# FearL0rd/ComfyUI-ParallelAnything

Hardware: AMD Instinct MI355X
Metric: images_per_s (whole-job; sec/it in ms_per_step), flux 1024^2 batch=8 (higher is better)
Workload: dtype bf16; 1 GPU; model=FLUX.1-dev-class MMDiT 12B, global_batch=8, resolution=1024, seq_len=4608, parallelism=dp1

## Files before the change

comfyui_parallelanything_amd/models/layers.py:

```python
from __future__ import annotations

import math
from dataclasses import dataclass
from typing import Tuple

import torch
from torch import nn

from .. import ops


class FusedGELU(nn.Module):

    def forward(self, x):
        return ops.gelu_tanh(x)


class GELULinear(nn.Module):

    def __init__(self, in_features: int, out_features: int):
        super().__init__()
        self.lin = nn.Linear(in_features, out_features, bias=True)

    def forward(self, x):
# ... 287 lines not shown
            qkv = qkv_lin.mm_fp8(x8, s_used)
            y_up = mlp_lin.mm_fp8(x8, s_used)
            if (hasattr(self.linear2_mlp, "gelu_quant")
                    and ops.hip_available("gelu_fp8")):
                mlp_fp8 = self.linear2_mlp.gelu_quant(y_up)
                mlp_act = None
            else:
                mlp_act = ops.gelu_tanh(y_up)
        else:
            x_in = ops.layer_norm_mod(x, mod.scale, mod.shift)
            qkv = self.linear1_qkv(x_in)
            mlp_act = self.linear1_mlp(x_in)
        qkv = qkv.unflatten(-1, (3, self.num_heads, -1))
        q, k, v = qkv.unbind(2)
        ops.qk_norm_rope_(
            q, k, self.norm.query_norm.scale, self.norm.key_norm.scale, pe
        )
        attn = ops.attention_bshd(q, k, v, self.attn.scale,
                                  key_mask=key_mask).flatten(2)
        if mlp_fp8 is not None:
            out = self.linear2_attn(attn) + self.linear2_mlp.mm_fp8(*mlp_fp8)
        elif x.is_cuda and isinstance(self.linear2_mlp, nn.Linear):
            acc = self.linear2_attn(attn).reshape(-1, hidden)
            out = torch.addmm(
                acc, mlp_act.reshape(-1, self.mlp_dim),
                self.linear2_mlp.weight.t(),
            ).reshape(B, S, hidden)
        else:
            out = self.linear2_attn(attn) + self.linear2_mlp(mlp_act)
        return ops.gate_residual(x, mod.gate, out)


class LastLayer(nn.Module):

    def __init__(self, hidden: int, out_dim: int):
        super().__init__()
        self.ada_lin = nn.Linear(hidden, 2 * hidden, bias=True)
        self.linear = nn.Linear(hidden, out_dim, bias=True)

    def forward(self, x, vec):
        shift, scale = self.ada_lin(torch.nn.functional.silu(vec)).chunk(2, dim=-1)
        return self.linear(ops.layer_norm_mod(x, scale, shift))


def _mod_outs(chunked):
    return ModOut(*chunked[:3]), (ModOut(*chunked[3:]) if len(chunked) == 6 else None)


# ... 31 lines not shown
```

comfyui_parallelanything_amd/ops/__init__.py:

```python
from __future__ import annotations

import glob
import importlib.util
import logging
import math
import os
from dataclasses import dataclass
from typing import Optional

import torch

from . import reference

log = logging.getLogger("parallelanything.ops")

_EXT = None
_EXT_TRIED = False
_ALLOW_EAGER = os.environ.get("PA_ALLOW_EAGER", "0") == "1"
_WARNED: set = set()
_NATIVE16 = (torch.bfloat16, torch.float16)


def _load_ext():
    global _EXT, _EXT_TRIED
# ... 107 lines not shown
    _refuse_unless(img.device == txt.device,
                   f"{op}: img is on {img.device}, txt on {txt.device}")
    for name, w in zip(("wq_t", "wk_t", "wq_i", "wk_i"), weights):
        _check_norm_weight(op, name, w, D, txt)
    _check_cs(op, cs, T + img.shape[1], D, txt)



def rms_norm(x: torch.Tensor, weight=None, eps: float = 1e-6) -> torch.Tensor:
    if x.is_cuda:
        ext = _require_ext("rms_norm")
        if ext is not None:
            return ext.rms_norm(x.contiguous(),
                                weight.contiguous() if weight is not None else None,
                                eps)
    return reference.rms_norm(x, weight, eps)


def layer_norm_mod(x, scale, shift, eps: float = 1e-6) -> torch.Tensor:
    if x.is_cuda:
        ext = _require_ext("layer_norm_mod")
        if ext is not None:
            if scale.dim() == x.dim() - 1:
                return ext.layer_norm_mod(
                    x.contiguous(), scale.contiguous(), shift.contiguous(), eps
                )
            _unsupported("layer_norm_mod", "per-token modulation")
    return reference.layer_norm_mod(x, scale, shift, eps)


def gate_residual(residual, gate, x) -> torch.Tensor:
    if x.dim() == 3 and gate.dim() == 2 and not x.is_cuda:
        _refuse_unless(
            tuple(gate.shape) == (x.shape[0], x.shape[2]),
            f"gate_residual: gate must be [B, D] = [{x.shape[0]}, "
            f"{x.shape[2]}], got {list(gate.shape)}")
        _refuse_unless(
            residual.shape == x.shape,
            f"gate_residual: residual {list(residual.shape)} must have x's "
            f"shape {list(x.shape)}")
        _refuse_unless(residual.dtype == x.dtype and gate.dtype == x.dtype,
                       "gate_residual: residual and gate dtypes must match "
                       "x's")
    if x.is_cuda:
        ext = _require_ext("gate_residual")
        if ext is not None and gate.dim() == x.dim() - 1:
            return ext.gate_residual(residual.contiguous(), gate.contiguous(),
                                     x.contiguous())
    return reference.gate_residual(residual, gate, x)


def group_norm_silu(x, num_groups: int, weight=None, bias=None,
                    eps: float = 1e-6) -> torch.Tensor:
    if x.is_cuda:
        ext = _require_ext("group_norm_silu")
        if ext is not None:
            if x.dim() == 4 and (x.shape[1] % num_groups) == 0:
                return ext.group_norm_silu(
                    x.contiguous(), int(num_groups),
                    weight.contiguous() if weight is not None else None,
                    bias.contiguous() if bias is not None else None,
                    eps,
                )
            _unsupported("group_norm_silu", f"dim={x.dim()}")
    return reference.group_norm_silu(x, num_groups, weight, bias, eps)


_GN_NHWC_MAX_C = 4096
_GN_NHWC_MAX_GROUPS = 256

# ... 448 lines not shown
```

comfyui_parallelanything_amd/ops/hip/common.h:

```cpp
#pragma once

#include <torch/extension.h>
#include <vector>
#include <ATen/ATen.h>
#include <c10/hip/HIPStream.h>

#include <hip/hip_runtime.h>
#include <hip/hip_bf16.h>
#include <hip/hip_fp16.h>
#include <hip/hip_fp8.h>

#define PA_DEV __device__ __forceinline__

using bf16 = __hip_bfloat16;
typedef __attribute__((ext_vector_type(8))) short short8;
typedef __attribute__((ext_vector_type(4))) short short4v;
typedef __attribute__((ext_vector_type(2))) float f32x2;

static constexpr int WAVE = 64;

PA_DEV float bf2f(bf16 v) { return __bfloat162float(v); }
PA_DEV bf16 f2bf(float v) { return __float2bfloat16(v); }

typedef __attribute__((ext_vector_type(16))) float f32x16;
// ... 76 lines not shown

static bool is_elem16(at::ScalarType t) {
    return t == at::kBFloat16 || t == at::kHalf;
}

#define PA_WITH_ELEM16(ST, ...)                                               \
    do {                                                                      \
        if ((ST) == at::kBFloat16) { using E = bf16; __VA_ARGS__; }           \
        else { using E = _Float16; __VA_ARGS__; }                             \
    } while (0)

#define PA_WITH_DTYPE(OP, ST, ...)                                            \
    do {                                                                      \
        if ((ST) == at::kBFloat16) { using T = bf16; __VA_ARGS__; }           \
        else if ((ST) == at::kHalf) { using T = _Float16; __VA_ARGS__; }      \
        else if ((ST) == at::kFloat) { using T = float; __VA_ARGS__; }        \
        else TORCH_CHECK(false, OP ": unsupported dtype ", (ST),              \
                         " (bf16, fp16 or fp32)");                            \
    } while (0)

static int grid_1d(long n) {
    return (int)std::min<long>((n + 255) / 256, 4096);
}
```

comfyui_parallelanything_amd/ops/hip/elementwise.h:

```cpp
#pragma once

template <typename T>
__global__ void gate_residual_kernel(const T* __restrict__ res,
                                     const T* __restrict__ gate,
                                     const T* __restrict__ x,
                                     T* __restrict__ out,
                                     long total, int S, int D) {
    const long stride = (long)gridDim.x * blockDim.x;
    for (long i = (long)blockIdx.x * blockDim.x + threadIdx.x; i < total; i += stride) {
        const long d = i % D;
        const long b = i / ((long)S * D);
        out[i] = (T)((float)res[i] + (float)gate[b * D + d] * (float)x[i]);
    }
}

template <typename E>
__global__ void gate_residual_vec_kernel(const E* __restrict__ res,
                                         const E* __restrict__ gate,
                                         const E* __restrict__ x,
                                         E* __restrict__ out,
                                         long total8, int S, int DV) {
    using EL = Elem16<E>;
    const long stride = (long)gridDim.x * blockDim.x;
    const short8* rv = reinterpret_cast<const short8*>(res);
    const short8* gv = reinterpret_cast<const short8*>(gate);
    const short8* xv = reinterpret_cast<const short8*>(x);
    short8* ov = reinterpret_cast<short8*>(out);
    for (long i = (long)blockIdx.x * blockDim.x + threadIdx.x; i < total8;
         i += stride) {
        const long dv = i % DV;
        const long b = i / ((long)S * DV);
        short8 r = rv[i], g = gv[b * DV + dv], xx = xv[i], o;
#pragma unroll
        for (int j = 0; j < 8; ++j) {
            float f = EL::ld((unsigned short)r[j]) +
                      EL::ld((unsigned short)g[j]) *
                          EL::ld((unsigned short)xx[j]);
            o[j] = (short)EL::st(f);
        }
        ov[i] = o;
    }
}

at::Tensor gate_residual(at::Tensor res, at::Tensor gate, at::Tensor x) {
    CHECK_GPU(x);
    TORCH_CHECK(x.dim() == 3 && gate.dim() == 2,
                "gate_residual: x [B,S,D], gate [B,D]");
    TORCH_CHECK(gate.size(0) == x.size(0) && gate.size(1) == x.size(2),
                "gate_residual: gate must be [B, D] = [", x.size(0), ", ",
                x.size(2), "], got ", gate.sizes());
    TORCH_CHECK(res.sizes() == x.sizes(), "gate_residual: residual ",
                res.sizes(), " must have x's shape ", x.sizes());
    CHECK_SAME_DEVICE(res, x);
    CHECK_SAME_DEVICE(gate, x);
    CHECK_SAME_DTYPE(res, x);
    CHECK_SAME_DTYPE(gate, x);
    if (x.numel() == 0) return at::empty(x.sizes(), x.options());
    auto rc = res.contiguous();
    auto gc = gate.contiguous();
    auto xc = x.contiguous();
    auto out = at::empty_like(xc);
    const long total = xc.numel();
    const int S = (int)xc.size(1), D = (int)xc.size(2);
    const int blocks = grid_1d(total);
    const auto st = xc.scalar_type();
    if (is_elem16(st) && (D % 8) == 0) {
        PA_WITH_ELEM16(st, hipLaunchKernelGGL(
            gate_residual_vec_kernel<E>, dim3(blocks), dim3(256), 0,
            cur_stream(), (const E*)rc.data_ptr(), (const E*)gc.data_ptr(),
            (const E*)xc.data_ptr(), (E*)out.data_ptr(), total / 8, S, D / 8));
    } else {
        PA_WITH_DTYPE("gate_residual", st, hipLaunchKernelGGL(
            gate_residual_kernel<T>, dim3(blocks), dim3(256), 0,
            cur_stream(), (const T*)rc.data_ptr(), (const T*)gc.data_ptr(),
            (const T*)xc.data_ptr(), (T*)out.data_ptr(), total, S, D));
    }
    return out;
}

template <bool kTail = false>
PA_DEV float gelu_tanh_f32(float f) {
    const float c = 0.7978845608028654f * (f + 0.044715f * f * f * f);
    const float En = __builtin_amdgcn_exp2f(-2.8853900817779268f * fabsf(c));
    const float r = __builtin_amdgcn_rcpf(1.f + En);
    return f * (c >= 0.f ? r : (kTail ? En * r : 1.f - r));
}

template <typename E>
__global__ void gelu_tanh_vec_kernel(const E* __restrict__ x,
                                     E* __restrict__ out, long total8,
                                     long rows, long w8, long in_stride8) {
    using EL = Elem16<E>;
    const long stride = (long)gridDim.x * blockDim.x;
    const short8* xv = reinterpret_cast<const short8*>(x);
    short8* ov = reinterpret_cast<short8*>(out);
    for (long i = (long)blockIdx.x * blockDim.x + threadIdx.x; i < total8;
         i += stride) {
        const long src = (in_stride8 == w8)
// ... 198 lines not shown
```

comfyui_parallelanything_amd/ops/hip/norm.h:

```cpp
#pragma once

template <typename T>
__global__ void rms_norm_kernel(const T* __restrict__ x, const T* __restrict__ w,
                                T* __restrict__ out, int D, float eps) {
    const long row = blockIdx.x;
    const T* xr = x + row * (long)D;
    T* yr = out + row * (long)D;
    __shared__ float scratch[8];

    float acc = 0.f;
    for (int i = threadIdx.x; i < D; i += blockDim.x) {
        float v = (float)xr[i];
        acc += v * v;
    }
    float ssq = block_reduce_sum<256>(acc, scratch);
    const float rrms = rsqrtf(ssq / (float)D + eps);
    for (int i = threadIdx.x; i < D; i += blockDim.x) {
        float v = (float)xr[i] * rrms;
        if (w != nullptr) v *= (float)w[i];
        yr[i] = (T)v;
    }
}

template <typename E>
// ... 98 lines not shown
        PA_WITH_ELEM16(st, hipLaunchKernelGGL(
            rms_norm_row_kernel<E>, dim3((unsigned)((rows + 3) / 4)),
            dim3(256), 0, cur_stream(), (const E*)xc.data_ptr(),
            (const E*)wptr, (E*)out.data_ptr(), rows, D, (float)eps));
    } else if (is_elem16(st) && (D % 8) == 0) {
        PA_WITH_ELEM16(st, hipLaunchKernelGGL(
            rms_norm_vec_kernel<E>, dim3((unsigned)rows), dim3(256), 0,
            cur_stream(), (const E*)xc.data_ptr(), (const E*)wptr,
            (E*)out.data_ptr(), D, (float)eps));
    } else {
        PA_WITH_DTYPE("rms_norm", st, hipLaunchKernelGGL(
            rms_norm_kernel<T>, dim3((unsigned)rows), dim3(256), 0,
            cur_stream(), (const T*)xc.data_ptr(), (const T*)wptr,
            (T*)out.data_ptr(), D, (float)eps));
    }
    return out;
}

template <typename T>
__global__ void layer_norm_mod_kernel(const T* __restrict__ x,
                                      const T* __restrict__ scale,
                                      const T* __restrict__ shift,
                                      T* __restrict__ out,
                                      int S, int D, float eps) {
    const long row = blockIdx.x;
    const long b = row / S;
    const T* xr = x + row * (long)D;
    const T* sc = scale + b * (long)D;
    const T* sh = shift + b * (long)D;
    T* yr = out + row * (long)D;
    __shared__ float scratch[8];

    float s1 = 0.f, s2 = 0.f;
    for (int i = threadIdx.x; i < D; i += blockDim.x) {
        float v = (float)xr[i];
        s1 += v;
        s2 += v * v;
    }
    float mean = block_reduce_sum<256>(s1, scratch) / (float)D;
    float var = block_reduce_sum<256>(s2, scratch) / (float)D - mean * mean;
    float corr = 0.f;
    if constexpr (sizeof(T) == 4) {
        float sd = 0.f, sq = 0.f;
        for (int i = threadIdx.x; i < D; i += blockDim.x) {
            float d = (float)xr[i] - mean;
            sd += d;
            sq += d * d;
        }
        corr = block_reduce_sum<256>(sd, scratch) / (float)D;
        var = block_reduce_sum<256>(sq, scratch) / (float)D - corr * corr;
    }
    const float rstd = rsqrtf(fmaxf(var, 0.f) + eps);
// ... 47 lines not shown
    }
    __syncthreads();
    s1 = (scratch[0] + scratch[2]) + (scratch[4] + scratch[6]);
    s2 = (scratch[1] + scratch[3]) + (scratch[5] + scratch[7]);
    const double inv_d = 1.0 / (double)D;
    const double m = s1 * inv_d;
    mean = (float)m;
    rstd = rsqrtf(fmaxf((float)(s2 * inv_d - m * m), 0.f) + eps);
}

template <typename EL>
PA_DEV float ln_modulate(short x, short scale, short shift, float mean,
                         float rstd) {
    float f = (EL::ld((unsigned short)x) - mean) * rstd;
    return f * (1.f + EL::ld((unsigned short)scale)) +
           EL::ld((unsigned short)shift);
}

template <typename E>
__global__ void layer_norm_mod_vec_kernel(const E* __restrict__ x,
                                          const E* __restrict__ scale,
                                          const E* __restrict__ shift,
                                          E* __restrict__ out,
                                          int S, int D, float eps) {
    using EL = Elem16<E>;
    const long row = blockIdx.x;
    const long b = row / S;
    const short8* xr = reinterpret_cast<const short8*>(x + row * (long)D);
    const short8* sc = reinterpret_cast<const short8*>(scale + b * (long)D);
    const short8* sh = reinterpret_cast<const short8*>(shift + b * (long)D);
    short8* yr = reinterpret_cast<short8*>(out + row * (long)D);
    const int DV = D / 8;
    __shared__ float scratch[8];

    float mean, rstd;
    ln_row_stats<EL>(xr, D, eps, scratch, mean, rstd);
    for (int i = threadIdx.x; i < DV; i += blockDim.x) {
        short8 v = xr[i], a = sc[i], c = sh[i], o;
#pragma unroll
        for (int j = 0; j < 8; ++j)
            o[j] = (short)EL::st(ln_modulate<EL>(v[j], a[j], c[j], mean, rstd));
        yr[i] = o;
    }
}

at::Tensor layer_norm_mod(at::Tensor x, at::Tensor scale, at::Tensor shift,
                          double eps) {
    CHECK_GPU(x);
    TORCH_CHECK(x.dim() == 3, "layer_norm_mod expects [B, S, D]");
    auto xc = x.contiguous();
    auto sc = scale.contiguous();
    auto sh = shift.contiguous();
    TORCH_CHECK(sc.sizes() == sh.sizes() && sc.dim() == 2, "scale/shift [B, D]");
    auto out = at::empty_like(xc);
    const int B = (int)xc.size(0), S = (int)xc.size(1), D = (int)xc.size(2);
    dim3 grid((unsigned)((long)B * S));
    const auto st = xc.scalar_type();
    CHECK_SAME_DTYPE(scale, x);
    CHECK_SAME_DTYPE(shift, x);
    if (is_elem16(st) && (D % 8) == 0) {
        PA_WITH_ELEM16(st, hipLaunchKernelGGL(
            layer_norm_mod_vec_kernel<E>, grid, dim3(256), 0, cur_stream(),
            (const E*)xc.data_ptr(), (const E*)sc.data_ptr(),
            (const E*)sh.data_ptr(), (E*)out.data_ptr(), S, D, (float)eps));
    } else {
        PA_WITH_DTYPE("layer_norm_mod", st, hipLaunchKernelGGL(
            layer_norm_mod_kernel<T>, grid, dim3(256), 0, cur_stream(),
            (const T*)xc.data_ptr(), (const T*)sc.data_ptr(),
            (const T*)sh.data_ptr(), (T*)out.data_ptr(), S, D, (float)eps));
    }
    return out;
}

template <typename T>
__global__ void group_norm_silu_kernel(const T* __restrict__ x,
                                       const float* __restrict__ w,
                                       const float* __restrict__ bias,
                                       T* __restrict__ out,
                                       int C, long HW, int G, float eps) {
    const int b = blockIdx.x / G;
    const int g = blockIdx.x % G;
    const int cpg = C / G;
    const long base = ((long)b * C + (long)g * cpg) * HW;
    const long n = (long)cpg * HW;
    __shared__ float scratch[8];

    float s1 = 0.f, s2 = 0.f;
    for (long i = threadIdx.x; i < n; i += blockDim.x) {
        float v = (float)x[base + i];
        s1 += v;
        s2 += v * v;
    }
// ... 51 lines not shown
```

comfyui_parallelanything_amd/ops/hip/qk_pack.h:

```cpp
#pragma once

template <typename EL>
PA_DEV unsigned int rms_rope_pair(unsigned int u, float w0, float w1, float c,
                                  float s, bool act, int D, float eps) {
    float a0 = EL::ld((unsigned short)(u & 0xffff));
    float a1 = EL::ld((unsigned short)(u >> 16));
    const float ss = wave_reduce_sum(act ? a0 * a0 + a1 * a1 : 0.f);
    const float rr = rsqrtf(ss / (float)D + eps);
    a0 = a0 * rr * w0;
    a1 = a1 * rr * w1;
    return (unsigned int)EL::st(a0 * c - a1 * s) |
           ((unsigned int)EL::st(a0 * s + a1 * c) << 16);
}

static void check_cs_table(const char* op, const at::Tensor& cs, long S, long D,
                           const at::Tensor& ref) {
    TORCH_CHECK(cs.dim() == 3 && cs.size(0) == S && cs.size(1) == D / 2 &&
                cs.size(2) == 2, op, ": cs must be [S, D/2, 2] = [", S, ", ",
                D / 2, ", 2], got ", cs.sizes());
    TORCH_CHECK(cs.device() == ref.device(), op, ": cs is on ", cs.device(),
                ", the activations on ", ref.device());
}

static void check_norm_weight(const char* op, const char* name,
                              const at::Tensor& w, long D,
                              const at::Tensor& ref) {
    TORCH_CHECK(w.dim() == 1 && w.size(0) == D, op, ": ", name,
                " must be [D] = [", D, "], got ", w.sizes());
    TORCH_CHECK(w.scalar_type() == ref.scalar_type(), op, ": ", name,
                " dtype (", w.scalar_type(), ") must match the activations (",
                ref.scalar_type(), ")");
    TORCH_CHECK(w.device() == ref.device(), op, ": ", name, " is on ",
                w.device(), ", the activations on ", ref.device());
}

template <typename E>
__global__ void qk_norm_rope_kernel(E* __restrict__ q, E* __restrict__ k,
                                    const E* __restrict__ wq,
                                    const E* __restrict__ wk,
                                    const float* __restrict__ cs,
                                    int S, int H, int D,
                                    long q_bs, long q_hs, long q_ss,
                                    long k_bs, long k_hs, long k_ss,
                                    long n_rows, float eps) {
    using EL = Elem16<E>;
    constexpr int RPW = 4;
    const int lane = threadIdx.x & 63;
    const long wave = ((long)blockIdx.x * blockDim.x + threadIdx.x) >> 6;
    const int pairs = D / 2;
    const bool act = lane < pairs;
    const int ln = act ? lane : 0;

    unsigned int uq[RPW], uk[RPW];
    unsigned int* qp[RPW];
    unsigned int* kp[RPW];
    float cvec[RPW], svec[RPW];
    const unsigned int uwq = reinterpret_cast<const unsigned int*>(wq)[ln];
    const unsigned int uwk = reinterpret_cast<const unsigned int*>(wk)[ln];
#pragma unroll
    for (int i = 0; i < RPW; ++i) {
        const long row = wave * RPW + i;
        const long rr = row < n_rows ? row : n_rows - 1;
        const long b = rr / ((long)S * H);
        const long sh = rr % ((long)S * H);
        const int sj = (int)(sh / H);
        const int h = (int)(sh % H);
        qp[i] = reinterpret_cast<unsigned int*>(
            q + b * q_bs + (long)sj * q_ss + (long)h * q_hs);
        kp[i] = reinterpret_cast<unsigned int*>(
            k + b * k_bs + (long)sj * k_ss + (long)h * k_hs);
        uq[i] = qp[i][ln];
        uk[i] = kp[i][ln];
        cvec[i] = cs[((long)sj * pairs + ln) * 2 + 0];
        svec[i] = cs[((long)sj * pairs + ln) * 2 + 1];
    }
    const float wq0 = EL::ld((unsigned short)(uwq & 0xffff));
    const float wq1 = EL::ld((unsigned short)(uwq >> 16));
    const float wk0 = EL::ld((unsigned short)(uwk & 0xffff));
    const float wk1 = EL::ld((unsigned short)(uwk >> 16));
#pragma unroll
    for (int i = 0; i < RPW; ++i) {
        if (wave * RPW + i >= n_rows) break;
        const unsigned int oq = rms_rope_pair<EL>(
            uq[i], wq0, wq1, cvec[i], svec[i], act, D, eps);
        if (act) qp[i][lane] = oq;
        const unsigned int ok = rms_rope_pair<EL>(
            uk[i], wk0, wk1, cvec[i], svec[i], act, D, eps);
        if (act) kp[i][lane] = ok;
    }
}

void qk_norm_rope_(at::Tensor q, at::Tensor k, at::Tensor wq, at::Tensor wk,
                   at::Tensor cs, double eps) {
    CHECK_GPU(q);
    TORCH_CHECK(q.dim() == 4 && k.dim() == 4, "qk_norm_rope_: [B,S,H,D] views");
    TORCH_CHECK(is_elem16(q.scalar_type()),
                "qk_norm_rope_: bf16 or fp16 only, got ", q.scalar_type());
    CHECK_SAME_DTYPE(k, q);
    CHECK_SAME_DEVICE(k, q);
    const int B = (int)q.size(0), S = (int)q.size(1), H = (int)q.size(2),
              D = (int)q.size(3);
    TORCH_CHECK(D % 2 == 0 && D <= 128, "qk_norm_rope_: D must be even, <=128");
    TORCH_CHECK(k.sizes() == q.sizes(), "qk_norm_rope_: k ", k.sizes(),
                " must have q's shape ", q.sizes());
    check_norm_weight("qk_norm_rope_", "wq", wq, D, q);
    check_norm_weight("qk_norm_rope_", "wk", wk, D, q);
    check_cs_table("qk_norm_rope_", cs, S, D, q);
    const long rows = (long)B * S * H;
    if (rows == 0 || D == 0) return;
    TORCH_CHECK(q.stride(3) == 1 && k.stride(3) == 1,
                "qk_norm_rope_: last dim contiguous");
    auto csf = cs.to(at::kFloat).contiguous();
    auto wqc = wq.contiguous();
    auto wkc = wk.contiguous();
    const long blocks = (((rows + 3) / 4) * 64 + 255) / 256;
    PA_WITH_ELEM16(q.scalar_type(), hipLaunchKernelGGL(
        qk_norm_rope_kernel<E>, dim3((unsigned)blocks), dim3(256), 0,
        cur_stream(), (E*)q.data_ptr(), (E*)k.data_ptr(),
        (const E*)wqc.data_ptr(), (const E*)wkc.data_ptr(),
        csf.data_ptr<float>(), S, H, D,
        q.stride(0), q.stride(2), q.stride(1),
        k.stride(0), k.stride(2), k.stride(1), rows, (float)eps));
}

template <typename E>
__global__ void pack_joint_qkv_kernel(
    const E* __restrict__ txt, const E* __restrict__ img,
    const E* __restrict__ wq_t, const E* __restrict__ wk_t,
    const E* __restrict__ wq_i, const E* __restrict__ wk_i,
    const float* __restrict__ cs,
    E* __restrict__ oq, E* __restrict__ ok, E* __restrict__ ov,
    int T, int Si, int H, int D,
    long t_bs, long t_ss, long t_qs, long t_hs,
    long i_bs, long i_ss, long i_qs, long i_hs,
    long n_rows, float eps) {
    using EL = Elem16<E>;
    constexpr int RPW = 4;
    const int lane = threadIdx.x & 63;
    const long wave = ((long)blockIdx.x * blockDim.x + threadIdx.x) >> 6;
    const int S = T + Si;
    const int pairs = D / 2;
    const bool act = lane < pairs;
    const int ln = act ? lane : 0;

    unsigned int uq[RPW], uk[RPW], uv[RPW], uwq[RPW], uwk[RPW];
    long obase[RPW];
    float cvec[RPW], svec[RPW];
#pragma unroll
    for (int i = 0; i < RPW; ++i) {
        const long row = wave * RPW + i;
        const long rr = row < n_rows ? row : n_rows - 1;
        const long b = rr / ((long)S * H);
        const long sh = rr % ((long)S * H);
        const int sj = (int)(sh / H);
        const int h = (int)(sh % H);
        const bool is_txt = sj < T;
        const E* src = is_txt
            ? txt + b * t_bs + (long)sj * t_ss + (long)h * t_hs
            : img + b * i_bs + (long)(sj - T) * i_ss + (long)h * i_hs;
        const long qs = is_txt ? t_qs : i_qs;
        uq[i] = reinterpret_cast<const unsigned int*>(src)[ln];
        uk[i] = reinterpret_cast<const unsigned int*>(src + qs)[ln];
        uv[i] = reinterpret_cast<const unsigned int*>(src + 2 * qs)[ln];
        uwq[i] = reinterpret_cast<const unsigned int*>(is_txt ? wq_t : wq_i)[ln];
        uwk[i] = reinterpret_cast<const unsigned int*>(is_txt ? wk_t : wk_i)[ln];
        cvec[i] = cs[((long)sj * pairs + ln) * 2 + 0];
        svec[i] = cs[((long)sj * pairs + ln) * 2 + 1];
        obase[i] = (((long)b * S + sj) * H + h) * (D / 2);
    }
#pragma unroll
    for (int i = 0; i < RPW; ++i) {
        if (wave * RPW + i >= n_rows) break;
        const unsigned int rq = rms_rope_pair<EL>(
            uq[i], EL::ld((unsigned short)(uwq[i] & 0xffff)),
            EL::ld((unsigned short)(uwq[i] >> 16)), cvec[i], svec[i], act, D,
            eps);
        if (act) reinterpret_cast<unsigned int*>(oq)[obase[i] + lane] = rq;
        const unsigned int rk = rms_rope_pair<EL>(
            uk[i], EL::ld((unsigned short)(uwk[i] & 0xffff)),
            EL::ld((unsigned short)(uwk[i] >> 16)), cvec[i], svec[i], act, D,
            eps);
        if (act) reinterpret_cast<unsigned int*>(ok)[obase[i] + lane] = rk;
        if (act) reinterpret_cast<unsigned int*>(ov)[obase[i] + lane] = uv[i];
    }
}

std::vector<at::Tensor> pack_joint_qkv(at::Tensor txt_qkv, at::Tensor img_qkv,
                                       at::Tensor wq_t, at::Tensor wk_t,
                                       at::Tensor wq_i, at::Tensor wk_i,
                                       at::Tensor cs, double eps) {
    CHECK_GPU(txt_qkv);
    TORCH_CHECK(txt_qkv.dim() == 5 && img_qkv.dim() == 5,
                "pack_joint_qkv expects [B,S,3,H,D] views");
    TORCH_CHECK(is_elem16(txt_qkv.scalar_type()),
                "pack_joint_qkv: bf16 or fp16 only, got ",
                txt_qkv.scalar_type());
    CHECK_SAME_DTYPE(img_qkv, txt_qkv);
    CHECK_SAME_DEVICE(img_qkv, txt_qkv);
    const int B = (int)txt_qkv.size(0), T = (int)txt_qkv.size(1),
              H = (int)txt_qkv.size(3), D = (int)txt_qkv.size(4);
    const int Si = (int)img_qkv.size(1);
    TORCH_CHECK(D % 2 == 0 && D <= 128,
                "pack_joint_qkv: D must be even and <= 128");
    TORCH_CHECK(txt_qkv.size(2) == 3 && img_qkv.size(2) == 3 &&
                img_qkv.size(0) == B && img_qkv.size(3) == H &&
                img_qkv.size(4) == D,
                "pack_joint_qkv: txt [B,T,3,H,D] and img [B,Si,3,H,D] must "
                "share B, H and D, got txt ", txt_qkv.sizes(), ", img ",
                img_qkv.sizes());
    check_norm_weight("pack_joint_qkv", "wq_t", wq_t, D, txt_qkv);
    check_norm_weight("pack_joint_qkv", "wk_t", wk_t, D, txt_qkv);
    check_norm_weight("pack_joint_qkv", "wq_i", wq_i, D, txt_qkv);
    check_norm_weight("pack_joint_qkv", "wk_i", wk_i, D, txt_qkv);
    check_cs_table("pack_joint_qkv", cs, (long)T + Si, D, txt_qkv);
    TORCH_CHECK(txt_qkv.numel() == 0 || txt_qkv.stride(4) == 1,
                "pack_joint_qkv: txt last dim contiguous");
    TORCH_CHECK(img_qkv.numel() == 0 || img_qkv.stride(4) == 1,
                "pack_joint_qkv: img last dim contiguous");
    auto csf = cs.to(at::kFloat).contiguous();
    auto opts = txt_qkv.options();
    auto oq = at::empty({B, T + Si, H, D}, opts);
    auto ok = at::empty({B, T + Si, H, D}, opts);
    auto ov = at::empty({B, T + Si, H, D}, opts);
    const long rows = (long)B * (T + Si) * H;
    if (rows == 0 || D == 0) return {oq, ok, ov};
    const long blocks = (((rows + 3) / 4) * 64 + 255) / 256;
    auto wqtc = wq_t.contiguous(), wktc = wk_t.contiguous();
    auto wqic = wq_i.contiguous(), wkic = wk_i.contiguous();
    PA_WITH_ELEM16(txt_qkv.scalar_type(), hipLaunchKernelGGL(
        pack_joint_qkv_kernel<E>, dim3((unsigned)blocks), dim3(256),
        0, cur_stream(),
        (const E*)txt_qkv.data_ptr(), (const E*)img_qkv.data_ptr(),
        (const E*)wqtc.data_ptr(), (const E*)wktc.data_ptr(),
        (const E*)wqic.data_ptr(), (const E*)wkic.data_ptr(),
        csf.data_ptr<float>(),
        (E*)oq.data_ptr(), (E*)ok.data_ptr(), (E*)ov.data_ptr(),
        T, Si, H, D,
        txt_qkv.stride(0), txt_qkv.stride(1), txt_qkv.stride(2),
        txt_qkv.stride(3),
        img_qkv.stride(0), img_qkv.stride(1), img_qkv.stride(2),
        img_qkv.stride(3),
        rows, (float)eps));
    return {oq, ok, ov};
}
```

Measured before the change: 15.33 images/s.

## Vectorize QK norm-RoPE per token and avoid contiguous copies of modulation tensors

Adds token-major QK RMS-norm+RoPE kernels (and a joint QKV pack variant) that load 8 elements per lane and reduce across lanes with DPP/swizzle, replacing the old one-pair-per-lane row kernel when layouts allow. Layer-norm modulation and gate-residual kernels now take a row stride, so strided scale/shift/gate views no longer need a contiguous copy. The final linear2 accumulation switches to in-place addmm_ to skip one output allocation. The risks are extra code paths for alignment and stride checks, and a small numeric-order change in the reduction.

After: 15.65 images/s (median of 6 runs). 2.1% higher.

```diff
diff --git a/comfyui_parallelanything_amd/models/layers.py b/comfyui_parallelanything_amd/models/layers.py
--- a/comfyui_parallelanything_amd/models/layers.py
+++ b/comfyui_parallelanything_amd/models/layers.py
@@ -333,8 +333,8 @@
             out = self.linear2_attn(attn) + self.linear2_mlp.mm_fp8(*mlp_fp8)
         elif x.is_cuda and isinstance(self.linear2_mlp, nn.Linear):
             acc = self.linear2_attn(attn).reshape(-1, hidden)
-            out = torch.addmm(
-                acc, mlp_act.reshape(-1, self.mlp_dim),
+            out = acc.addmm_(
+                mlp_act.reshape(-1, self.mlp_dim),
                 self.linear2_mlp.weight.t(),
             ).reshape(B, S, hidden)
         else:
diff --git a/comfyui_parallelanything_amd/ops/__init__.py b/comfyui_parallelanything_amd/ops/__init__.py
--- a/comfyui_parallelanything_amd/ops/__init__.py
+++ b/comfyui_parallelanything_amd/ops/__init__.py
@@ -153,9 +153,7 @@
         ext = _require_ext("layer_norm_mod")
         if ext is not None:
             if scale.dim() == x.dim() - 1:
-                return ext.layer_norm_mod(
-                    x.contiguous(), scale.contiguous(), shift.contiguous(), eps
-                )
+                return ext.layer_norm_mod(x.contiguous(), scale, shift, eps)
             _unsupported("layer_norm_mod", "per-token modulation")
     return reference.layer_norm_mod(x, scale, shift, eps)
 
@@ -176,7 +174,7 @@
     if x.is_cuda:
         ext = _require_ext("gate_residual")
         if ext is not None and gate.dim() == x.dim() - 1:
-            return ext.gate_residual(residual.contiguous(), gate.contiguous(),
+            return ext.gate_residual(residual.contiguous(), gate,
                                      x.contiguous())
     return reference.gate_residual(residual, gate, x)
 
diff --git a/comfyui_parallelanything_amd/ops/hip/common.h b/comfyui_parallelanything_amd/ops/hip/common.h
--- a/comfyui_parallelanything_amd/ops/hip/common.h
+++ b/comfyui_parallelanything_amd/ops/hip/common.h
@@ -122,3 +122,11 @@
 static int grid_1d(long n) {
     return (int)std::min<long>((n + 255) / 256, 4096);
 }
+
+static at::Tensor mod_rows(const at::Tensor& t, bool vec) {
+    bool ok = t.dim() == 2 && (t.size(1) <= 1 || t.stride(1) == 1);
+    if (ok && vec)
+        ok = (reinterpret_cast<uintptr_t>(t.data_ptr()) % 16) == 0 &&
+             (t.size(0) <= 1 || (t.stride(0) * t.element_size()) % 16 == 0);
+    return ok ? t : t.contiguous();
+}
diff --git a/comfyui_parallelanything_amd/ops/hip/elementwise.h b/comfyui_parallelanything_amd/ops/hip/elementwise.h
--- a/comfyui_parallelanything_amd/ops/hip/elementwise.h
+++ b/comfyui_parallelanything_amd/ops/hip/elementwise.h
@@ -5,12 +5,12 @@
                                      const T* __restrict__ gate,
                                      const T* __restrict__ x,
                                      T* __restrict__ out,
-                                     long total, int S, int D) {
+                                     long total, int S, int D, long g_rs) {
     const long stride = (long)gridDim.x * blockDim.x;
     for (long i = (long)blockIdx.x * blockDim.x + threadIdx.x; i < total; i += stride) {
         const long d = i % D;
         const long b = i / ((long)S * D);
-        out[i] = (T)((float)res[i] + (float)gate[b * D + d] * (float)x[i]);
+        out[i] = (T)((float)res[i] + (float)gate[b * g_rs + d] * (float)x[i]);
     }
 }
 
@@ -19,7 +19,8 @@
                                          const E* __restrict__ gate,
                                          const E* __restrict__ x,
                                          E* __restrict__ out,
-                                         long total8, int S, int DV) {
+                                         long total8, int S, int DV,
+                                         long g_rsv) {
     using EL = Elem16<E>;
     const long stride = (long)gridDim.x * blockDim.x;
     const short8* rv = reinterpret_cast<const short8*>(res);
@@ -30,7 +31,7 @@
          i += stride) {
         const long dv = i % DV;
         const long b = i / ((long)S * DV);
-        short8 r = rv[i], g = gv[b * DV + dv], xx = xv[i], o;
+        short8 r = rv[i], g = gv[b * g_rsv + dv], xx = xv[i], o;
 #pragma unroll
         for (int j = 0; j < 8; ++j) {
             float f = EL::ld((unsigned short)r[j]) +
@@ -57,23 +58,26 @@
     CHECK_SAME_DTYPE(gate, x);
     if (x.numel() == 0) return at::empty(x.sizes(), x.options());
     auto rc = res.contiguous();
-    auto gc = gate.contiguous();
     auto xc = x.contiguous();
     auto out = at::empty_like(xc);
     const long total = xc.numel();
     const int S = (int)xc.size(1), D = (int)xc.size(2);
     const int blocks = grid_1d(total);
     const auto st = xc.scalar_type();
-    if (is_elem16(st) && (D % 8) == 0) {
+    const bool vec = is_elem16(st) && (D % 8) == 0;
+    auto gc = mod_rows(gate, vec);
+    const long g_rs = gc.stride(0);
+    if (vec) {
         PA_WITH_ELEM16(st, hipLaunchKernelGGL(
             gate_residual_vec_kernel<E>, dim3(blocks), dim3(256), 0,
             cur_stream(), (const E*)rc.data_ptr(), (const E*)gc.data_ptr(),
-            (const E*)xc.data_ptr(), (E*)out.data_ptr(), total / 8, S, D / 8));
+            (const E*)xc.data_ptr(), (E*)out.data_ptr(), total / 8, S, D / 8,
+            g_rs / 8));
     } else {
         PA_WITH_DTYPE("gate_residual", st, hipLaunchKernelGGL(
             gate_residual_kernel<T>, dim3(blocks), dim3(256), 0,
             cur_stream(), (const T*)rc.data_ptr(), (const T*)gc.data_ptr(),
-            (const T*)xc.data_ptr(), (T*)out.data_ptr(), total, S, D));
+            (const T*)xc.data_ptr(), (T*)out.data_ptr(), total, S, D, g_rs));
     }
     return out;
 }
diff --git a/comfyui_parallelanything_amd/ops/hip/norm.h b/comfyui_parallelanything_amd/ops/hip/norm.h
--- a/comfyui_parallelanything_amd/ops/hip/norm.h
+++ b/comfyui_parallelanything_amd/ops/hip/norm.h
@@ -144,12 +144,13 @@
                                       const T* __restrict__ scale,
                                       const T* __restrict__ shift,
                                       T* __restrict__ out,
-                                      int S, int D, float eps) {
+                                      int S, int D, long sc_rs, long sh_rs,
+                                      float eps) {
     const long row = blockIdx.x;
     const long b = row / S;
     const T* xr = x + row * (long)D;
-    const T* sc = scale + b * (long)D;
-    const T* sh = shift + b * (long)D;
+    const T* sc = scale + b * sc_rs;
+    const T* sh = shift + b * sh_rs;
     T* yr = out + row * (long)D;
     __shared__ float scratch[8];
 
@@ -243,13 +244,14 @@
                                           const E* __restrict__ scale,
                                           const E* __restrict__ shift,
                                           E* __restrict__ out,
-                                          int S, int D, float eps) {
+                                          int S, int D, long sc_rs,
+                                          long sh_rs, float eps) {
     using EL = Elem16<E>;
     const long row = blockIdx.x;
     const long b = row / S;
     const short8* xr = reinterpret_cast<const short8*>(x + row * (long)D);
-    const short8* sc = reinterpret_cast<const short8*>(scale + b * (long)D);
-    const short8* sh = reinterpret_cast<const short8*>(shift + b * (long)D);
+    const short8* sc = reinterpret_cast<const short8*>(scale + b * sc_rs);
+    const short8* sh = reinterpret_cast<const short8*>(shift + b * sh_rs);
     short8* yr = reinterpret_cast<short8*>(out + row * (long)D);
     const int DV = D / 8;
     __shared__ float scratch[8];
@@ -270,25 +272,36 @@
     CHECK_GPU(x);
     TORCH_CHECK(x.dim() == 3, "layer_norm_mod expects [B, S, D]");
     auto xc = x.contiguous();
-    auto sc = scale.contiguous();
-    auto sh = shift.contiguous();
-    TORCH_CHECK(sc.sizes() == sh.sizes() && sc.dim() == 2, "scale/shift [B, D]");
+    TORCH_CHECK(scale.sizes() == shift.sizes() && scale.dim() == 2,
+                "scale/shift [B, D]");
     auto out = at::empty_like(xc);
     const int B = (int)xc.size(0), S = (int)xc.size(1), D = (int)xc.size(2);
+    TORCH_CHECK(scale.size(0) == B && scale.size(1) == D,
+                "layer_norm_mod: scale/shift must be [B, D] = [", B, ", ", D,
+                "], got ", scale.sizes());
     dim3 grid((unsigned)((long)B * S));
     const auto st = xc.scalar_type();
     CHECK_SAME_DTYPE(scale, x);
     CHECK_SAME_DTYPE(shift, x);
-    if (is_elem16(st) && (D % 8) == 0) {
+    CHECK_SAME_DEVICE(scale, x);
+    CHECK_SAME_DEVICE(shift, x);
+    if (xc.numel() == 0) return out;
+    const bool vec = is_elem16(st) && (D % 8) == 0;
+    auto sc = mod_rows(scale, vec);
+    auto sh = mod_rows(shift, vec);
+    const long sc_rs = sc.stride(0), sh_rs = sh.stride(0);
+    if (vec) {
         PA_WITH_ELEM16(st, hipLaunchKernelGGL(
             layer_norm_mod_vec_kernel<E>, grid, dim3(256), 0, cur_stream(),
             (const E*)xc.data_ptr(), (const E*)sc.data_ptr(),
-            (const E*)sh.data_ptr(), (E*)out.data_ptr(), S, D, (float)eps));
+            (const E*)sh.data_ptr(), (E*)out.data_ptr(), S, D, sc_rs, sh_rs,
+            (float)eps));
     } else {
         PA_WITH_DTYPE("layer_norm_mod", st, hipLaunchKernelGGL(
             layer_norm_mod_kernel<T>, grid, dim3(256), 0, cur_stream(),
             (const T*)xc.data_ptr(), (const T*)sc.data_ptr(),
-            (const T*)sh.data_ptr(), (T*)out.data_ptr(), S, D, (float)eps));
+            (const T*)sh.data_ptr(), (T*)out.data_ptr(), S, D, sc_rs, sh_rs,
+            (float)eps));
     }
     return out;
 }
diff --git a/comfyui_parallelanything_amd/ops/hip/qk_pack.h b/comfyui_parallelanything_amd/ops/hip/qk_pack.h
--- a/comfyui_parallelanything_amd/ops/hip/qk_pack.h
+++ b/comfyui_parallelanything_amd/ops/hip/qk_pack.h
@@ -1,17 +1,6 @@
 #pragma once
 
-template <typename EL>
-PA_DEV unsigned int rms_rope_pair(unsigned int u, float w0, float w1, float c,
-                                  float s, bool act, int D, float eps) {
-    float a0 = EL::ld((unsigned short)(u & 0xffff));
-    float a1 = EL::ld((unsigned short)(u >> 16));
-    const float ss = wave_reduce_sum(act ? a0 * a0 + a1 * a1 : 0.f);
-    const float rr = rsqrtf(ss / (float)D + eps);
-    a0 = a0 * rr * w0;
-    a1 = a1 * rr * w1;
-    return (unsigned int)EL::st(a0 * c - a1 * s) |
-           ((unsigned int)EL::st(a0 * s + a1 * c) << 16);
-}
+#include "qk_pack_kernels.h"
 
 static void check_cs_table(const char* op, const at::Tensor& cs, long S, long D,
                            const at::Tensor& ref) {
@@ -34,60 +23,25 @@
                 w.device(), ", the activations on ", ref.device());
 }
 
-template <typename E>
-__global__ void qk_norm_rope_kernel(E* __restrict__ q, E* __restrict__ k,
-                                    const E* __restrict__ wq,
-                                    const E* __restrict__ wk,
-                                    const float* __restrict__ cs,
-                                    int S, int H, int D,
-                                    long q_bs, long q_hs, long q_ss,
-                                    long k_bs, long k_hs, long k_ss,
-                                    long n_rows, float eps) {
-    using EL = Elem16<E>;
-    constexpr int RPW = 4;
-    const int lane = threadIdx.x & 63;
-    const long wave = ((long)blockIdx.x * blockDim.x + threadIdx.x) >> 6;
-    const int pairs = D / 2;
-    const bool act = lane < pairs;
-    const int ln = act ? lane : 0;
+static bool ptr16(const at::Tensor& t) {
+    return (reinterpret_cast<uintptr_t>(t.data_ptr()) % 16) == 0;
+}
 
-    unsigned int uq[RPW], uk[RPW];
-    unsigned int* qp[RPW];
-    unsigned int* kp[RPW];
-    float cvec[RPW], svec[RPW];
-    const unsigned int uwq = reinterpret_cast<const unsigned int*>(wq)[ln];
-    const unsigned int uwk = reinterpret_cast<const unsigned int*>(wk)[ln];
-#pragma unroll
-    for (int i = 0; i < RPW; ++i) {
-        const long row = wave * RPW + i;
-        const long rr = row < n_rows ? row : n_rows - 1;
-        const long b = rr / ((long)S * H);
-        const long sh = rr % ((long)S * H);
-        const int sj = (int)(sh / H);
-        const int h = (int)(sh % H);
-        qp[i] = reinterpret_cast<unsigned int*>(
-            q + b * q_bs + (long)sj * q_ss + (long)h * q_hs);
-        kp[i] = reinterpret_cast<unsigned int*>(
-            k + b * k_bs + (long)sj * k_ss + (long)h * k_hs);
-        uq[i] = qp[i][ln];
-        uk[i] = kp[i][ln];
-        cvec[i] = cs[((long)sj * pairs + ln) * 2 + 0];
-        svec[i] = cs[((long)sj * pairs + ln) * 2 + 1];
-    }
-    const float wq0 = EL::ld((unsigned short)(uwq & 0xffff));
-    const float wq1 = EL::ld((unsigned short)(uwq >> 16));
-    const float wk0 = EL::ld((unsigned short)(uwk & 0xffff));
-    const float wk1 = EL::ld((unsigned short)(uwk >> 16));
-#pragma unroll
-    for (int i = 0; i < RPW; ++i) {
-        if (wave * RPW + i >= n_rows) break;
-        const unsigned int oq = rms_rope_pair<EL>(
-            uq[i], wq0, wq1, cvec[i], svec[i], act, D, eps);
-        if (act) qp[i][lane] = oq;
-        const unsigned int ok = rms_rope_pair<EL>(
-            uk[i], wk0, wk1, cvec[i], svec[i], act, D, eps);
-        if (act) kp[i][lane] = ok;
-    }
+static bool tok_major(const at::Tensor& t, int tok_dim, int h_dim, long D) {
+    if (!ptr16(t)) return false;
+    if (t.size(h_dim) > 1 && t.stride(h_dim) != D) return false;
+    for (int d = 0; d <= tok_dim; ++d)
+        if (t.size(d) > 1 && (t.stride(d) % 8) != 0) return false;
+    return true;
+}
+
+static constexpr int QK_TOK_CH = 2;
+
+static std::pair<unsigned, unsigned> tok_work(long tokens, long HD) {
+    const long nchunk = (HD + QK_TOK_CH * 512 - 1) / (QK_TOK_CH * 512);
+    const long waves = tokens * nchunk;
+    if (HD >= (1L << 30) || waves >= (1L << 31) - 4) return {0u, 0u};
+    return {(unsigned)nchunk, (unsigned)waves};
 }
 
 void qk_norm_rope_(at::Tensor q, at::Tensor k, at::Tensor wq, at::Tensor wk,
@@ -113,6 +67,21 @@
     auto csf = cs.to(at::kFloat).contiguous();
     auto wqc = wq.contiguous();
     auto wkc = wk.contiguous();
+    const auto work = tok_work((long)B * S, (long)H * D);
+    if ((D == 128 || D == 64) && work.first != 0 && tok_major(q, 1, 2, D) &&
+        tok_major(k, 1, 2, D) && ptr16(csf) && ptr16(wqc) && ptr16(wkc)) {
+#define PA_QK_TOK(DT)                                                         \
+        PA_WITH_ELEM16(q.scalar_type(), hipLaunchKernelGGL(                   \
+            (qk_norm_rope_tok_kernel<E, DT, QK_TOK_CH, true>),                \
+            dim3((work.second + 3) / 4), dim3(256), 0, cur_stream(),          \
+            (E*)q.data_ptr(), (E*)k.data_ptr(), (const E*)wqc.data_ptr(),     \
+            (const E*)wkc.data_ptr(), csf.data_ptr<float>(), (unsigned)S,     \
+            H * D, D, q.stride(0), q.stride(1), k.stride(0), k.stride(1),     \
+            work.first, work.second, (float)eps))
+        if (D == 128) PA_QK_TOK(128); else PA_QK_TOK(64);
+#undef PA_QK_TOK
+        return;
+    }
     const long blocks = (((rows + 3) / 4) * 64 + 255) / 256;
     PA_WITH_ELEM16(q.scalar_type(), hipLaunchKernelGGL(
         qk_norm_rope_kernel<E>, dim3((unsigned)blocks), dim3(256), 0,
@@ -121,68 +90,6 @@
         csf.data_ptr<float>(), S, H, D,
         q.stride(0), q.stride(2), q.stride(1),
         k.stride(0), k.stride(2), k.stride(1), rows, (float)eps));
-}
-
-template <typename E>
-__global__ void pack_joint_qkv_kernel(
-    const E* __restrict__ txt, const E* __restrict__ img,
-    const E* __restrict__ wq_t, const E* __restrict__ wk_t,
-    const E* __restrict__ wq_i, const E* __restrict__ wk_i,
-    const float* __restrict__ cs,
-    E* __restrict__ oq, E* __restrict__ ok, E* __restrict__ ov,
-    int T, int Si, int H, int D,
-    long t_bs, long t_ss, long t_qs, long t_hs,
-    long i_bs, long i_ss, long i_qs, long i_hs,
-    long n_rows, float eps) {
-    using EL = Elem16<E>;
-    constexpr int RPW = 4;
-    const int lane = threadIdx.x & 63;
-    const long wave = ((long)blockIdx.x * blockDim.x + threadIdx.x) >> 6;
-    const int S = T + Si;
-    const int pairs = D / 2;
-    const bool act = lane < pairs;
-    const int ln = act ? lane : 0;
-
-    unsigned int uq[RPW], uk[RPW], uv[RPW], uwq[RPW], uwk[RPW];
-    long obase[RPW];
-    float cvec[RPW], svec[RPW];
-#pragma unroll
-    for (int i = 0; i < RPW; ++i) {
-        const long row = wave * RPW + i;
-        const long rr = row < n_rows ? row : n_rows - 1;
-        const long b = rr / ((long)S * H);
-        const long sh = rr % ((long)S * H);
-        const int sj = (int)(sh / H);
-        const int h = (int)(sh % H);
-        const bool is_txt = sj < T;
-        const E* src = is_txt
-            ? txt + b * t_bs + (long)sj * t_ss + (long)h * t_hs
-            : img + b * i_bs + (long)(sj - T) * i_ss + (long)h * i_hs;
-        const long qs = is_txt ? t_qs : i_qs;
-        uq[i] = reinterpret_cast<const unsigned int*>(src)[ln];
-        uk[i] = reinterpret_cast<const unsigned int*>(src + qs)[ln];
-        uv[i] = reinterpret_cast<const unsigned int*>(src + 2 * qs)[ln];
-        uwq[i] = reinterpret_cast<const unsigned int*>(is_txt ? wq_t : wq_i)[ln];
-        uwk[i] = reinterpret_cast<const unsigned int*>(is_txt ? wk_t : wk_i)[ln];
-        cvec[i] = cs[((long)sj * pairs + ln) * 2 + 0];
-        svec[i] = cs[((long)sj * pairs + ln) * 2 + 1];
-        obase[i] = (((long)b * S + sj) * H + h) * (D / 2);
-    }
-#pragma unroll
-    for (int i = 0; i < RPW; ++i) {
-        if (wave * RPW + i >= n_rows) break;
-        const unsigned int rq = rms_rope_pair<EL>(
-            uq[i], EL::ld((unsigned short)(uwq[i] & 0xffff)),
-            EL::ld((unsigned short)(uwq[i] >> 16)), cvec[i], svec[i], act, D,
-            eps);
-        if (act) reinterpret_cast<unsigned int*>(oq)[obase[i] + lane] = rq;
-        const unsigned int rk = rms_rope_pair<EL>(
-            uk[i], EL::ld((unsigned short)(uwk[i] & 0xffff)),
-            EL::ld((unsigned short)(uwk[i] >> 16)), cvec[i], svec[i], act, D,
-            eps);
-        if (act) reinterpret_cast<unsigned int*>(ok)[obase[i] + lane] = rk;
-        if (act) reinterpret_cast<unsigned int*>(ov)[obase[i] + lane] = uv[i];
-    }
 }
 
 std::vector<at::Tensor> pack_joint_qkv(at::Tensor txt_qkv, at::Tensor img_qkv,
@@ -224,9 +131,31 @@
     auto ov = at::empty({B, T + Si, H, D}, opts);
     const long rows = (long)B * (T + Si) * H;
     if (rows == 0 || D == 0) return {oq, ok, ov};
-    const long blocks = (((rows + 3) / 4) * 64 + 255) / 256;
     auto wqtc = wq_t.contiguous(), wktc = wk_t.contiguous();
     auto wqic = wq_i.contiguous(), wkic = wk_i.contiguous();
+    const auto work = tok_work((long)B * (T + Si), (long)H * D);
+    const bool t_ok = T == 0 || tok_major(txt_qkv, 2, 3, D);
+    const bool i_ok = Si == 0 || tok_major(img_qkv, 2, 3, D);
+    if ((D == 128 || D == 64) && work.first != 0 && t_ok && i_ok &&
+        ptr16(csf) && ptr16(wqtc) && ptr16(wktc) && ptr16(wqic) &&
+        ptr16(wkic) && ptr16(oq) && ptr16(ok) && ptr16(ov)) {
+#define PA_PACK_TOK(DT)                                                       \
+        PA_WITH_ELEM16(txt_qkv.scalar_type(), hipLaunchKernelGGL(             \
+            (pack_joint_qkv_tok_kernel<E, DT, QK_TOK_CH, true>),              \
+            dim3((work.second + 3) / 4), dim3(256), 0, cur_stream(),          \
+            (const E*)txt_qkv.data_ptr(), (const E*)img_qkv.data_ptr(),       \
+            (const E*)wqtc.data_ptr(), (const E*)wktc.data_ptr(),             \
+            (const E*)wqic.data_ptr(), (const E*)wkic.data_ptr(),             \
+            csf.data_ptr<float>(), (E*)oq.data_ptr(), (E*)ok.data_ptr(),      \
+            (E*)ov.data_ptr(), (unsigned)T, (unsigned)(T + Si), H * D, D,     \
+            txt_qkv.stride(0), txt_qkv.stride(1), txt_qkv.stride(2),          \
+            img_qkv.stride(0), img_qkv.stride(1), img_qkv.stride(2),          \
+            work.first, work.second, (float)eps))
+        if (D == 128) PA_PACK_TOK(128); else PA_PACK_TOK(64);
+#undef PA_PACK_TOK
+        return {oq, ok, ov};
+    }
+    const long blocks = (((rows + 3) / 4) * 64 + 255) / 256;
     PA_WITH_ELEM16(txt_qkv.scalar_type(), hipLaunchKernelGGL(
         pack_joint_qkv_kernel<E>, dim3((unsigned)blocks), dim3(256),
         0, cur_stream(),
diff --git a/comfyui_parallelanything_amd/ops/hip/qk_pack_kernels.h b/comfyui_parallelanything_amd/ops/hip/qk_pack_kernels.h
--- /dev/null
+++ b/comfyui_parallelanything_amd/ops/hip/qk_pack_kernels.h
@@ -0,0 +1,304 @@
+#pragma once
+
+template <typename EL>
+PA_DEV unsigned int rms_rope_pair(unsigned int u, float w0, float w1, float c,
+                                  float s, bool act, int D, float eps) {
+    float a0 = EL::ld((unsigned short)(u & 0xffff));
+    float a1 = EL::ld((unsigned short)(u >> 16));
+    const float ss = wave_reduce_sum(act ? a0 * a0 + a1 * a1 : 0.f);
+    const float rr = rsqrtf(ss / (float)D + eps);
+    a0 = a0 * rr * w0;
+    a1 = a1 * rr * w1;
+    return (unsigned int)EL::st(a0 * c - a1 * s) |
+           ((unsigned int)EL::st(a0 * s + a1 * c) << 16);
+}
+
+template <typename E>
+__global__ void qk_norm_rope_kernel(E* __restrict__ q, E* __restrict__ k,
+                                    const E* __restrict__ wq,
+                                    const E* __restrict__ wk,
+                                    const float* __restrict__ cs,
+                                    int S, int H, int D,
+                                    long q_bs, long q_hs, long q_ss,
+                                    long k_bs, long k_hs, long k_ss,
+                                    long n_rows, float eps) {
+    using EL = Elem16<E>;
+    constexpr int RPW = 4;
+    const int lane = threadIdx.x & 63;
+    const long wave = ((long)blockIdx.x * blockDim.x + threadIdx.x) >> 6;
+    const int pairs = D / 2;
+    const bool act = lane < pairs;
+    const int ln = act ? lane : 0;
+
+    unsigned int uq[RPW], uk[RPW];
+    unsigned int* qp[RPW];
+    unsigned int* kp[RPW];
+    float cvec[RPW], svec[RPW];
+    const unsigned int uwq = reinterpret_cast<const unsigned int*>(wq)[ln];
+    const unsigned int uwk = reinterpret_cast<const unsigned int*>(wk)[ln];
+#pragma unroll
+    for (int i = 0; i < RPW; ++i) {
+        const long row = wave * RPW + i;
+        const long rr = row < n_rows ? row : n_rows - 1;
+        const long b = rr / ((long)S * H);
+        const long sh = rr % ((long)S * H);
+        const int sj = (int)(sh / H);
+        const int h = (int)(sh % H);
+        qp[i] = reinterpret_cast<unsigned int*>(
+            q + b * q_bs + (long)sj * q_ss + (long)h * q_hs);
+        kp[i] = reinterpret_cast<unsigned int*>(
+            k + b * k_bs + (long)sj * k_ss + (long)h * k_hs);
+        uq[i] = qp[i][ln];
+        uk[i] = kp[i][ln];
+        cvec[i] = cs[((long)sj * pairs + ln) * 2 + 0];
+        svec[i] = cs[((long)sj * pairs + ln) * 2 + 1];
+    }
+    const float wq0 = EL::ld((unsigned short)(uwq & 0xffff));
+    const float wq1 = EL::ld((unsigned short)(uwq >> 16));
+    const float wk0 = EL::ld((unsigned short)(uwk & 0xffff));
+    const float wk1 = EL::ld((unsigned short)(uwk >> 16));
+#pragma unroll
+    for (int i = 0; i < RPW; ++i) {
+        if (wave * RPW + i >= n_rows) break;
+        const unsigned int oq = rms_rope_pair<EL>(
+            uq[i], wq0, wq1, cvec[i], svec[i], act, D, eps);
+        if (act) qp[i][lane] = oq;
+        const unsigned int ok = rms_rope_pair<EL>(
+            uk[i], wk0, wk1, cvec[i], svec[i], act, D, eps);
+        if (act) kp[i][lane] = ok;
+    }
+}
+
+template <typename E>
+__global__ void pack_joint_qkv_kernel(
+    const E* __restrict__ txt, const E* __restrict__ img,
+    const E* __restrict__ wq_t, const E* __restrict__ wk_t,
+    const E* __restrict__ wq_i, const E* __restrict__ wk_i,
+    const float* __restrict__ cs,
+    E* __restrict__ oq, E* __restrict__ ok, E* __restrict__ ov,
+    int T, int Si, int H, int D,
+    long t_bs, long t_ss, long t_qs, long t_hs,
+    long i_bs, long i_ss, long i_qs, long i_hs,
+    long n_rows, float eps) {
+    using EL = Elem16<E>;
+    constexpr int RPW = 4;
+    const int lane = threadIdx.x & 63;
+    const long wave = ((long)blockIdx.x * blockDim.x + threadIdx.x) >> 6;
+    const int S = T + Si;
+    const int pairs = D / 2;
+    const bool act = lane < pairs;
+    const int ln = act ? lane : 0;
+
+    unsigned int uq[RPW], uk[RPW], uv[RPW], uwq[RPW], uwk[RPW];
+    long obase[RPW];
+    float cvec[RPW], svec[RPW];
+#pragma unroll
+    for (int i = 0; i < RPW; ++i) {
+        const long row = wave * RPW + i;
+        const long rr = row < n_rows ? row : n_rows - 1;
+        const long b = rr / ((long)S * H);
+        const long sh = rr % ((long)S * H);
+        const int sj = (int)(sh / H);
+        const int h = (int)(sh % H);
+        const bool is_txt = sj < T;
+        const E* src = is_txt
+            ? txt + b * t_bs + (long)sj * t_ss + (long)h * t_hs
+            : img + b * i_bs + (long)(sj - T) * i_ss + (long)h * i_hs;
+        const long qs = is_txt ? t_qs : i_qs;
+        uq[i] = reinterpret_cast<const unsigned int*>(src)[ln];
+        uk[i] = reinterpret_cast<const unsigned int*>(src + qs)[ln];
+        uv[i] = reinterpret_cast<const unsigned int*>(src + 2 * qs)[ln];
+        uwq[i] = reinterpret_cast<const unsigned int*>(is_txt ? wq_t : wq_i)[ln];
+        uwk[i] = reinterpret_cast<const unsigned int*>(is_txt ? wk_t : wk_i)[ln];
+        cvec[i] = cs[((long)sj * pairs + ln) * 2 + 0];
+        svec[i] = cs[((long)sj * pairs + ln) * 2 + 1];
+        obase[i] = (((long)b * S + sj) * H + h) * (D / 2);
+    }
+#pragma unroll
+    for (int i = 0; i < RPW; ++i) {
+        if (wave * RPW + i >= n_rows) break;
+        const unsigned int rq = rms_rope_pair<EL>(
+            uq[i], EL::ld((unsigned short)(uwq[i] & 0xffff)),
+            EL::ld((unsigned short)(uwq[i] >> 16)), cvec[i], svec[i], act, D,
+            eps);
+        if (act) reinterpret_cast<unsigned int*>(oq)[obase[i] + lane] = rq;
+        const unsigned int rk = rms_rope_pair<EL>(
+            uk[i], EL::ld((unsigned short)(uwk[i] & 0xffff)),
+            EL::ld((unsigned short)(uwk[i] >> 16)), cvec[i], svec[i], act, D,
+            eps);
+        if (act) reinterpret_cast<unsigned int*>(ok)[obase[i] + lane] = rk;
+        if (act) reinterpret_cast<unsigned int*>(ov)[obase[i] + lane] = uv[i];
+    }
+}
+
+
+template <int M, bool kDpp>
+PA_DEV float row_xor(float v) {
+    if constexpr (!kDpp) {
+        return __shfl_xor(v, M, 64);
+    } else {
+        int i = __builtin_bit_cast(int, v);
+        if constexpr (M == 8)
+            i = __builtin_amdgcn_update_dpp(0, i, 0x128, 0xf, 0xf, true);
+        else if constexpr (M == 4)
+            i = __builtin_amdgcn_ds_swizzle(i, (4 << 10) | 0x1f);
+        else if constexpr (M == 2)
+            i = __builtin_amdgcn_update_dpp(0, i, 0x4e, 0xf, 0xf, true);
+        else
+            i = __builtin_amdgcn_update_dpp(0, i, 0xb1, 0xf, 0xf, true);
+        return __builtin_bit_cast(float, i);
+    }
+}
+
+template <typename EL>
+PA_DEV void ld8(short8 u, float (&f)[8]) {
+#pragma unroll
+    for (int j = 0; j < 8; ++j) f[j] = EL::ld((unsigned short)u[j]);
+}
+
+template <typename EL, int DT, bool kDpp>
+PA_DEV short8 rms_rope_vec8(short8 u, const float (&w)[8],
+                            const float (&cs)[8], int D, float eps) {
+#pragma clang fp contract(off)
+    float a[8], t[4];
+    ld8<EL>(u, a);
+#pragma unroll
+    for (int j = 0; j < 4; ++j) {
+        const float a0 = a[2 * j], a1 = a[2 * j + 1];
+        t[j] = a0 * a0 + a1 * a1;
+    }
+    if constexpr (DT == 128) {
+#pragma unroll
+        for (int j = 0; j < 4; ++j) t[j] += row_xor<8, kDpp>(t[j]);
+    }
+#pragma unroll
+    for (int j = 0; j < 4; ++j) t[j] += row_xor<4, kDpp>(t[j]);
+#pragma unroll
+    for (int j = 0; j < 4; ++j) t[j] += row_xor<2, kDpp>(t[j]);
+#pragma unroll
+    for (int j = 0; j < 4; ++j) t[j] += row_xor<1, kDpp>(t[j]);
+    const float ss = (t[0] + t[2]) + (t[1] + t[3]);
+    const float rr = rsqrtf(ss / (float)D + eps);
+    short8 o;
+#pragma unroll
+    for (int j = 0; j < 4; ++j) {
+        float a0 = a[2 * j], a1 = a[2 * j + 1];
+        const float c = cs[2 * j], s = cs[2 * j + 1];
+        a0 = a0 * rr * w[2 * j];
+        a1 = a1 * rr * w[2 * j + 1];
+        o[2 * j] = (short)EL::st(a0 * c - a1 * s);
+        o[2 * j + 1] = (short)EL::st(a0 * s + a1 * c);
+    }
+    return o;
+}
+
+template <int DT>
+PA_DEV void ld_cs8(const float* __restrict__ cs, unsigned s, int pos,
+                   float (&f)[8]) {
+    const float4* p =
+        reinterpret_cast<const float4*>(cs + (long)s * DT + pos);
+    const float4 x = p[0], y = p[1];
+    f[0] = x.x; f[1] = x.y; f[2] = x.z; f[3] = x.w;
+    f[4] = y.x; f[5] = y.y; f[6] = y.z; f[7] = y.w;
+}
+
+template <typename E, int DT, int CH, bool kDpp>
+__global__ void __launch_bounds__(256)
+qk_norm_rope_tok_kernel(E* __restrict__ q, E* __restrict__ k,
+                        const E* __restrict__ wq, const E* __restrict__ wk,
+                        const float* __restrict__ cs,
+                        unsigned S, int HD, int D, long q_bs, long q_ss,
+                        long k_bs, long k_ss, unsigned nchunk,
+                        unsigned n_work, float eps) {
+    using EL = Elem16<E>;
+    const int lane = threadIdx.x & 63;
+    const unsigned wave = __builtin_amdgcn_readfirstlane(
+        blockIdx.x * (blockDim.x >> 6) + (threadIdx.x >> 6));
+    if (wave >= n_work) return;
+    const unsigned tok = wave / nchunk, chunk = wave % nchunk;
+    const unsigned b = tok / S, s = tok % S;
+    const int pos = (lane * 8) % DT;
+    const int first = (int)chunk * (CH * 512);
+    E* qt = q + b * q_bs + s * q_ss;
+    E* kt = k + b * k_bs + s * k_ss;
+
+    short8 uq[CH], uk[CH];
+    int off[CH];
+#pragma unroll
+    for (int i = 0; i < CH; ++i) {
+        const int o = first + i * 512 + lane * 8;
+        off[i] = o < HD ? o : -1;
+        const int ol = o < HD ? o : pos;
+        uq[i] = *reinterpret_cast<const short8*>(qt + ol);
+        uk[i] = *reinterpret_cast<const short8*>(kt + ol);
+    }
+    float fwq[8], fwk[8], fcs[8];
+    ld8<EL>(*reinterpret_cast<const short8*>(wq + pos), fwq);
+    ld8<EL>(*reinterpret_cast<const short8*>(wk + pos), fwk);
+    ld_cs8<DT>(cs, s, pos, fcs);
+#pragma unroll
+    for (int i = 0; i < CH; ++i) {
+        if (first + i * 512 >= HD) break;
+        const short8 oq = rms_rope_vec8<EL, DT, kDpp>(uq[i], fwq, fcs, D, eps);
+        if (off[i] >= 0) *reinterpret_cast<short8*>(qt + off[i]) = oq;
+        const short8 ok = rms_rope_vec8<EL, DT, kDpp>(uk[i], fwk, fcs, D, eps);
+        if (off[i] >= 0) *reinterpret_cast<short8*>(kt + off[i]) = ok;
+    }
+}
+
+template <typename E, int DT, int CH, bool kDpp>
+__global__ void __launch_bounds__(256)
+pack_joint_qkv_tok_kernel(
+    const E* __restrict__ txt, const E* __restrict__ img,
+    const E* __restrict__ wq_t, const E* __restrict__ wk_t,
+    const E* __restrict__ wq_i, const E* __restrict__ wk_i,
+    const float* __restrict__ cs,
+    E* __restrict__ oq, E* __restrict__ ok, E* __restrict__ ov,
+    unsigned T, unsigned S, int HD, int D,
+    long t_bs, long t_ss, long t_qs,
+    long i_bs, long i_ss, long i_qs,
+    unsigned nchunk, unsigned n_work, float eps) {
+    using EL = Elem16<E>;
+    const int lane = threadIdx.x & 63;
+    const unsigned wave = __builtin_amdgcn_readfirstlane(
+        blockIdx.x * (blockDim.x >> 6) + (threadIdx.x >> 6));
+    if (wave >= n_work) return;
+    const unsigned tok = wave / nchunk, chunk = wave % nchunk;
+    const unsigned b = tok / S, s = tok % S;
+    const bool is_txt = s < T;
+    const int pos = (lane * 8) % DT;
+    const int first = (int)chunk * (CH * 512);
+    const E* src = is_txt ? txt + b * t_bs + s * t_ss
+                          : img + b * i_bs + (s - T) * i_ss;
+    const long qs = is_txt ? t_qs : i_qs;
+    const long obase = (long)tok * HD;
+
+    short8 uq[CH], uk[CH], uv[CH];
+    int off[CH];
+#pragma unroll
+    for (int i = 0; i < CH; ++i) {
+        const int o = first + i * 512 + lane * 8;
+        off[i] = o < HD ? o : -1;
+        const int ol = o < HD ? o : pos;
+        uq[i] = *reinterpret_cast<const short8*>(src + ol);
+        uk[i] = *reinterpret_cast<const short8*>(src + qs + ol);
+        uv[i] = *reinterpret_cast<const short8*>(src + 2 * qs + ol);
+    }
+    float fwq[8], fwk[8], fcs[8];
+    ld8<EL>(*reinterpret_cast<const short8*>((is_txt ? wq_t : wq_i) + pos),
+            fwq);
+    ld8<EL>(*reinterpret_cast<const short8*>((is_txt ? wk_t : wk_i) + pos),
+            fwk);
+    ld_cs8<DT>(cs, s, pos, fcs);
+#pragma unroll
+    for (int i = 0; i < CH; ++i) {
+        if (first + i * 512 >= HD) break;
+        const short8 rq = rms_rope_vec8<EL, DT, kDpp>(uq[i], fwq, fcs, D, eps);
+        const short8 rk = rms_rope_vec8<EL, DT, kDpp>(uk[i], fwk, fcs, D, eps);
+        if (off[i] >= 0) {
+            *reinterpret_cast<short8*>(oq + obase + off[i]) = rq;
+            *reinterpret_cast<short8*>(ok + obase + off[i]) = rk;
+            *reinterpret_cast<short8*>(ov + obase + off[i]) = uv[i];
+        }
+    }
+}
```
